# Lagrange-Labs/mapreduce-plonky2

Hardware: AMD Instinct MI355X
Metric: leaf proofs/sec (whole node) + NTT GB/s vs HBM peak, 2^20-row table build, 1/2/4/8 GPU (higher is better)
Workload: dtype u64 (Goldilocks field)

## Files before the change

mapreduce-plonky2_amd/csrc/poseidon.cuh:

```cuda
#pragma once
#include "gl.cuh"
#include "perm_constants.h"

#pragma push_macro("MP2G_DEVCONST")
#undef MP2G_DEVCONST
#undef MP2G_PERM_CONSTANTS_H
#define MP2G_DEVCONST static constexpr
namespace p2_cx {
#include "perm_constants.h"
constexpr u64 diag_shl32(int i) { return (u64)(((unsigned __int128)POSEIDON2_DIAG_M1[i] << 32) % GL_P); }
constexpr unsigned diag_narrow(int i = 0) {
  return i == 12 ? 0u : (GL_MULC_NARROW(POSEIDON2_DIAG_M1[i], diag_shl32(i)) ? 1u << i : 0u) | diag_narrow(i + 1);
}
}
#pragma pop_macro("MP2G_DEVCONST")
MP2G_DEVCONST uint64_t POSEIDON2_DIAG_M1_SHL32[12] = {
  p2_cx::diag_shl32(0), p2_cx::diag_shl32(1), p2_cx::diag_shl32(2), p2_cx::diag_shl32(3), p2_cx::diag_shl32(4), p2_cx::diag_shl32(5),
  p2_cx::diag_shl32(6), p2_cx::diag_shl32(7), p2_cx::diag_shl32(8), p2_cx::diag_shl32(9), p2_cx::diag_shl32(10), p2_cx::diag_shl32(11),
};
constexpr unsigned POSEIDON2_DIAG_NARROW = p2_cx::diag_narrow();
static_assert(POSEIDON2_DIAG_NARROW == 0xcfeu, "limbs 0, 8 and 9 take gl_mulc_addw's carry (profiles/p2_diag measured this split)");

#define MP2G_POSEIDON2 0
#define MP2G_POSEIDON 1

#define c_p2_ext POSEIDON2_RC_EXT
#define c_p2_int POSEIDON2_RC_INT
#define c_p2_diag POSEIDON2_DIAG_M1
#define c_p2_diag_shl32 POSEIDON2_DIAG_M1_SHL32
#define c_p_rc POSEIDON_RC

GLHD u64 p2_sbox(u64 x, u64 rc) {
  u64 t = gl_addw(x, rc);
  u64 t2 = gl_mulw(t, t), t4 = gl_mulw(t2, t2), t3 = gl_mulw(t, t2);
  return gl_mulw(t3, t4);
}
GLHD void p2_m4_plain(u64& a, u64& b, u64& c, u64& d) {
  u64 t0 = a + b, t1 = c + d;
  u64 t2 = (b << 1) + t1, t3 = (d << 1) + t0;
  u64 t4 = (t1 << 2) + t3, t5 = (t0 << 2) + t2;
  a = t3 + t5; b = t5; c = t2 + t4; d = t4;
}
GLHD void p2_external_half(u64 v[12]) {
  p2_m4_plain(v[0], v[1], v[2], v[3]);
  p2_m4_plain(v[4], v[5], v[6], v[7]);
  p2_m4_plain(v[8], v[9], v[10], v[11]);
#pragma unroll
  for (int i = 0; i < 4; i++) {
    u64 sum = v[i] + v[4 + i] + v[8 + i];
    v[i] += sum; v[4 + i] += sum; v[8 + i] += sum;
  }
}
template <bool RC>
GLHD void p2_external_rc(u64 s[12], const u64* rc) {
  u64 lo[12], hi[12];
#pragma unroll
  for (int i = 0; i < 12; i++) { lo[i] = (u32)s[i]; hi[i] = s[i] >> 32; }
  p2_external_half(lo);
  p2_external_half(hi);
#if defined(__HIP_DEVICE_COMPILE__)
#pragma unroll
  for (int i = 0; i < 12; i++) {
    u64 L = lo[i], H = hi[i];
    if (RC) { L += (u64)(u32)rc[i]; H += rc[i] >> 32; }
    H += L >> 32;
    s[i] = gl_reduce96w(gl_mk((u32)L, (u32)H), H >> 32);
  }
#else
#pragma unroll
  for (int i = 0; i < 12; i++) {
    u32 c0, c1, top = (u32)(hi[i] >> 32);
    u32 l0 = (u32)lo[i];
    u32 l1 = __builtin_addc((u32)(lo[i] >> 32), (u32)hi[i], 0u, &c0);
    top += c0;
    if (RC) {
      const u64 k = rc[i];
      l0 = __builtin_addc(l0, (u32)k, 0u, &c0);
      l1 = __builtin_addc(l1, (u32)(k >> 32), c0, &c1);
      top += c1;
    }
    s[i] = gl_reduce96w(gl_mk(l0, l1), top);
  }
#endif
}
GLHD void p2_external(u64 s[12]) { p2_external_rc<false>(s, nullptr); }
GLHD u64 p2_sbox0(u64 t) {
  u64 t2 = gl_mulw_k(t, t), t4 = gl_mulw_k(t2, t2), t3 = gl_mulw_k(t, t2);
  return gl_mulw_k(t3, t4);
}
GLHD u64 p2_diag_mul_addw(int i, u64 a, u64 c) {
  if ((POSEIDON2_DIAG_NARROW >> i) & 1) return gl_mulc_addw<true>(a, c_p2_diag[i], c_p2_diag_shl32[i], c);
  return gl_mulc_addw<false>(a, c_p2_diag[i], c_p2_diag_shl32[i], c);
}
GLD u64 p2_limb_sum(const u64 s[12]) {
#if defined(__HIP_DEVICE_COMPILE__)
  u64 w = s[0], ha, hb;
#pragma unroll
  for (int i = 1; i < 12; i++) w += s[i];
#define P2_MAD1_(r, x, z) asm volatile("v_mad_u64_u32 %0, vcc, %1, 1, %2" : "=v"(r) : "v"((u32)((x) >> 32)), "v"(z) : "vcc")
  asm volatile("v_mad_u64_u32 %0, vcc, %1, 1, 0" : "=v"(ha) : "v"((u32)(s[0] >> 32)) : "vcc");
  asm volatile("v_mad_u64_u32 %0, vcc, %1, 1, 0" : "=v"(hb) : "v"((u32)(s[1] >> 32)) : "vcc");
#pragma unroll
  for (int i = 2; i < 12; i += 2) {
    P2_MAD1_(ha, s[i], ha);
    P2_MAD1_(hb, s[i + 1], hb);
  }
  const u64 h = ha + hb;
  const u32 c = (u32)(w >> 32) - (u32)h;
  u64 t;
  asm volatile("v_mad_u64_u32 %0, vcc, %1, 1, %2" : "=v"(t) : "v"(c), "v"(h) : "vcc");
#undef P2_MAD1_
  return gl_reduce96w(w, t >> 32);
#else
  unsigned __int128 x = 0;
  for (int i = 0; i < 12; i++) x += s[i];
  return gl_reduce96w((u64)x, (u64)(x >> 64));
#endif
}
GLHD void p2_internal(u64 s[12]) {
#if defined(__HIP_DEVICE_COMPILE__)
  const u64 sum = p2_limb_sum(s);
#pragma unroll
  for (int i = 0; i < 12; i++) {
    s[i] = p2_diag_mul_addw(i, s[i], sum);
    __builtin_amdgcn_sched_barrier(0);
  }
#else
  u64 acc = s[0];
  u64 top = 0;
#pragma unroll
  for (int i = 1; i < 12; i++) {
    bool c = __builtin_add_overflow(acc, s[i], &acc);
    top += c ? 1 : 0;
  }
#pragma unroll
  for (int i = 0; i < 12; i++) {
    u64 lo, hi;
    gl_mul_wide(s[i], c_p2_diag[i], lo, hi);
    bool c = __builtin_add_overflow(lo, acc, &lo);
    s[i] = gl_reduce128w(lo, hi + top + (c ? 1 : 0));
  }
#endif
}
GLHD void poseidon2_perm(u64 s[12]) {
  p2_external_rc<true>(s, c_p2_ext);
#pragma unroll 1
  for (int r = 0; r < 4; r++) {
#pragma unroll
    for (int i = 0; i < 12; i++) s[i] = p2_sbox0(s[i]);
    if (r < 3) p2_external_rc<true>(s, c_p2_ext + 12 * (r + 1)); else p2_external(s);
  }
#pragma unroll 11
  for (int r = 0; r < 22; r++) {
    s[0] = p2_sbox0(gl_addw(s[0], c_p2_int[r]));
    p2_internal(s);
  }
#pragma unroll
  for (int i = 0; i < 12; i++) s[i] = gl_addw(s[i], c_p2_ext[48 + i]);
#pragma unroll 1
  for (int r = 4; r < 8; r++) {
#pragma unroll
    for (int i = 0; i < 12; i++) s[i] = p2_sbox0(s[i]);
    if (r < 7) p2_external_rc<true>(s, c_p2_ext + 12 * (r + 1)); else p2_external(s);
  }
#pragma unroll
  for (int i = 0; i < 12; i++) s[i] = gl_canon(s[i]);
}

template <bool RC>
GLHD void poseidon_mds_rc(u64 s[12], const u64* rc) {
  const u32 circ[12] = {17, 15, 41, 16, 2, 28, 13, 13, 39, 18, 34, 20};
  u64 lo[12], hi[12];
#pragma unroll
  for (int i = 0; i < 12; i++) { lo[i] = (u32)s[i]; hi[i] = s[i] >> 32; }
  u64 out[12];
#pragma unroll
  for (int r = 0; r < 12; r++) {
    u64 al = 0, ah = 0;
#pragma unroll
    for (int i = 0; i < 12; i++) {
      al += lo[(i + r) % 12] * circ[i];
      ah += hi[(i + r) % 12] * circ[i];
    }
    if (r == 0) { al += lo[0] * 8; ah += hi[0] * 8; }
    u32 c0, c1, top = (u32)(ah >> 32);
    u32 l0 = (u32)al;
    u32 l1 = __builtin_addc((u32)(al >> 32), (u32)ah, 0u, &c0);
    top += c0;
    if (RC) {
      const u64 k = rc[r];
      l0 = __builtin_addc(l0, (u32)k, 0u, &c0);
      l1 = __builtin_addc(l1, (u32)(k >> 32), c0, &c1);
      top += c1;
    }
    out[r] = gl_reduce96w(gl_mk(l0, l1), top);
  }
#pragma unroll
  for (int i = 0; i < 12; i++) s[i] = out[i];
}
GLHD void poseidon_mds(u64 s[12]) { poseidon_mds_rc<false>(s, nullptr); }
GLHD void poseidon_perm(u64 s[12]) {
#pragma unroll
  for (int i = 0; i < 12; i++) s[i] = gl_addw(s[i], c_p_rc[i]);
#pragma unroll 1
  for (int r = 0; r < 30; r++) {
    if (r < 4 || r >= 26) {
#pragma unroll
      for (int i = 0; i < 12; i++) s[i] = p2_sbox0(s[i]);
    } else {
      s[0] = p2_sbox0(s[0]);
    }
    if (r < 29) poseidon_mds_rc<true>(s, c_p_rc + 12 * (r + 1)); else poseidon_mds(s);
  }
#pragma unroll
  for (int i = 0; i < 12; i++) s[i] = gl_canon(s[i]);
}
template <int VARIANT>
GLHD void perm(u64 s[12]) {
  if (VARIANT == MP2G_POSEIDON2) poseidon2_perm(s); else poseidon_perm(s);
}
template <int VARIANT>
GLD void two_to_one(const u64 l[4], const u64 r[4], u64 out[4]) {
  u64 s[12];
#pragma unroll
  for (int i = 0; i < 4; i++) { s[i] = l[i]; s[4 + i] = r[i]; s[8 + i] = 0; }
  perm<VARIANT>(s);
#pragma unroll
  for (int i = 0; i < 4; i++) out[i] = s[i];
}
```

Measured before the change: 1036.

## Compute Poseidon2 external MDS carries via truncated 32-bit high-part estimate

Replaces the split lo/hi 64-bit limb evaluation of the external MDS on device with a wrapping 64-bit matrix applied directly to the state. The overflow word is recovered from a separate 32-bit matrix over truncated high bits (top 32-T bits), plus a rounding bias. This roughly halves the 64-bit add work in the external layer. The cost is a small extra u32 matrix pass and reliance on a bounded-error argument for correct carry recovery.

```diff
diff --git a/mapreduce-plonky2_amd/csrc/poseidon.cuh b/mapreduce-plonky2_amd/csrc/poseidon.cuh
--- a/mapreduce-plonky2_amd/csrc/poseidon.cuh
+++ b/mapreduce-plonky2_amd/csrc/poseidon.cuh
@@ -51,22 +51,45 @@
     v[i] += sum; v[4 + i] += sum; v[8 + i] += sum;
   }
 }
-template <bool RC>
+GLHD void p2_m4_u32(u32& a, u32& b, u32& c, u32& d) {
+  u32 t0 = a + b, t1 = c + d;
+  u32 t2 = (b << 1) + t1, t3 = (d << 1) + t0;
+  u32 t4 = (t1 << 2) + t3, t5 = (t0 << 2) + t2;
+  a = t3 + t5; b = t5; c = t2 + t4; d = t4;
+}
+GLHD void p2_external_half_u32(u32 v[12]) {
+  p2_m4_u32(v[0], v[1], v[2], v[3]);
+  p2_m4_u32(v[4], v[5], v[6], v[7]);
+  p2_m4_u32(v[8], v[9], v[10], v[11]);
+#pragma unroll
+  for (int i = 0; i < 4; i++) {
+    u32 sum = v[i] + v[4 + i] + v[8 + i];
+    v[i] += sum; v[4 + i] += sum; v[8 + i] += sum;
+  }
+}
+#define P2_EXT_TRUNC 16
+template <bool RC, int T = P2_EXT_TRUNC>
 GLHD void p2_external_rc(u64 s[12], const u64* rc) {
+#if defined(__HIP_DEVICE_COMPILE__)
+  static_assert(T >= 8 && T <= 24, "A_i + (hi32(rc_i) >> T) + 2^(31-T) < 2^32 needs T >= 7, 64 < 2^(31-T) needs T <= 24");
+  u32 a[12];
+#pragma unroll
+  for (int i = 0; i < 12; i++) a[i] = (u32)(s[i] >> 32) >> T;
+  p2_external_half_u32(a);
+  p2_external_half(s);
+#pragma unroll
+  for (int i = 0; i < 12; i++) {
+    u32 kc = 1u << (31 - T);
+    if (RC) { s[i] += rc[i]; kc += (u32)(rc[i] >> 32) >> T; }
+    const u32 k = (a[i] + kc - ((u32)(s[i] >> 32) >> T)) >> (32 - T);
+    s[i] = gl_reduce96w(s[i], k);
+  }
+#else
   u64 lo[12], hi[12];
 #pragma unroll
   for (int i = 0; i < 12; i++) { lo[i] = (u32)s[i]; hi[i] = s[i] >> 32; }
   p2_external_half(lo);
   p2_external_half(hi);
-#if defined(__HIP_DEVICE_COMPILE__)
-#pragma unroll
-  for (int i = 0; i < 12; i++) {
-    u64 L = lo[i], H = hi[i];
-    if (RC) { L += (u64)(u32)rc[i]; H += rc[i] >> 32; }
-    H += L >> 32;
-    s[i] = gl_reduce96w(gl_mk((u32)L, (u32)H), H >> 32);
-  }
-#else
 #pragma unroll
   for (int i = 0; i < 12; i++) {
     u32 c0, c1, top = (u32)(hi[i] >> 32);
```

After: 1043, median of 6. About the same (+0.7%).
